# biiiipy/JaxMARL-HFT

Hardware: AMD Instinct MI355X
Metric: env steps/sec (whole node), 2-agent MARL, 10-level LOB, NUM_ENVS=4096 (higher is better)
Workload: dtype int32

## Files before the change

### jaxmarl-hft_amd/csrc/hftlob.hip

```cpp
#include <hip/hip_runtime.h>
#include <stdint.h>
#include <string.h>
#include <stdio.h>
#include <mutex>
#include <type_traits>
#include <limits.h>

#include "../../include/hftlob.h"

typedef int32_t i32;
typedef uint32_t u32;
typedef uint8_t u8;
#define DEV __device__ __forceinline__

DEV int lane_id() { return __lane_id(); }
DEV i32 rdl(i32 v, int l) { return __builtin_amdgcn_readlane(v, l); }
DEV i32 wrl(i32 old, i32 val, int l) { return __lane_id() == l ? val : old; }
DEV i32 uni(i32 v) { return __builtin_amdgcn_readfirstlane(v); }
DEV float unif(float v) { return __int_as_float(__builtin_amdgcn_readfirstlane(__float_as_int(v))); }
DEV i32 wadd(i32 a, i32 b) { return (i32)((u32)a + (u32)b); }
DEV i32 wsub(i32 a, i32 b) { return (i32)((u32)a - (u32)b); }
DEV i32 wmul(i32 a, i32 b) { return (i32)((u32)a * (u32)b); }
DEV i32 iabs_(i32 a) { return a < 0 ? wsub(0, a) : a; }
DEV i32 isign(i32 a) { return (a > 0) - (a < 0); }
// ... 2370 lines not shown
}
DEV Key lane_key(Key v) { return Key{(u32)rdl((i32)v.a, 0), (u32)rdl((i32)v.b, 0)}; }
DEV Key from_lane(Key v, int src) {
    return Key{(u32)__builtin_amdgcn_ds_bpermute(src << 2, (i32)v.a), (u32)__builtin_amdgcn_ds_bpermute(src << 2, (i32)v.b)};
}
template <bool MD>
DEV StepKeys step_keys(const hftlob_env_cfg& c, int n_env, int e, const u32* keys, bool sampled, const Key& master) {
    const bool part = c.prng_partitionable;
    const int l = lane_id(), nTy = c.n_types, A = c.n_action_msgs;
    Key key;
    Key nm{0u, 0u};
    if (sampled) {
        const Key v = split_key(master, n_env + 1, l == 0 ? e + 1 : 0, part);
        key = lane_key(v);
        nm = Key{(u32)rdl((i32)v.a, 1), (u32)rdl((i32)v.b, 1)};
    } else {
        key = Key{keys[2 * e], keys[2 * e + 1]};
    }
    const bool two = part && c.n_agents <= 16 && A <= 32;
    const bool hi_lane = two && l >= 48;
    const int ag = l - (hi_lane ? 48 : 32);
    int t = 0, i = 0;
    agent_of_lane(c, ag < 0 ? 0 : ag, t, i);
    const bool agent_lane = (ag >= 0) & (ag < c.n_agents);
    const Key L1 = split_key(key, l < 2 ? 2 : nTy, l < 2 ? l : l - 2, part);
    StepKeys o;
    o.key = key;
    o.next_master = nm;
    o.k1 = Key{(u32)rdl((i32)L1.a, 0), (u32)rdl((i32)L1.b, 0)};
    o.key_reset = Key{(u32)rdl((i32)L1.a, 1), (u32)rdl((i32)L1.b, 1)};
    if (two) {
        const Key P2 = from_lane(L1, agent_lane ? 2 + t : 0);
        const Key L2 = split_key(P2, agent_lane ? type_n_agents(c, t) : 2, agent_lane ? i : 1, part);
        const Key L3 = split_key(L2, 2, ((l == 0) | hi_lane) ? 1 : 0, part);
        const Key sub = from_lane(L3, 0);
        const u32 bits = random_bits(l < A ? sub : L3, 1, l < A ? l : 0, part);
        o.shuffle_bits = bits;
        const u32 hb = bits, lb = (u32)__builtin_amdgcn_ds_bpermute(((l + 16) & 63) << 2, (i32)bits);
        const i32 na = agent_lane ? type_action_hi(c, t, MD) : 1;
        const u32 span = na <= 0 ? 1u : (u32)na;
        u32 mult = 65536u % span;
        mult = (mult * mult) % span;
        o.acts = (i32)(((hb % span) * mult + (lb % span)) % span);
        return o;
    }
    const Key P2 = from_lane(L1, agent_lane ? 2 + t : 0);
    const Key L2 = split_key(P2, agent_lane ? type_n_agents(c, t) : 2, agent_lane ? i : 1, part);
    const Key L3a = split_key(L2, 2, l == 0 ? 1 : 0, part);
    const Key L3b = split_key(L2, 2, 1, part);
    const Key sub = from_lane(L3a, 0);
    o.shuffle_bits = random_bits(sub, A > 0 ? A : 1, l < A ? l : 0, part);
    const u32 hb = random_bits(L3a, 1, 0, part), lb = random_bits(L3b, 1, 0, part);
    const i32 na = agent_lane ? type_action_hi(c, t, MD) : 1;
    const u32 span = na <= 0 ? 1u : (u32)na;
    u32 mult = 65536u % span;
    mult = (mult * mult) % span;
    o.acts = (i32)(((hb % span) * mult + (lb % span)) % span);
    return o;
}

#define KB_STEPS 4
__host__ __device__ inline bool kb_ok(const hftlob_env_cfg& c) {
    return c.prng_partitionable && c.n_agents <= 3 && c.n_action_msgs <= 8 && c.n_types <= 6 &&
           6 + c.n_agents + c.n_action_msgs <= 16;
}
__host__ __device__ inline int kb_words(const hftlob_env_cfg& c) { return 6 + c.n_agents + c.n_action_msgs; }
__host__ __device__ inline bool rows_in_trades(const hftlob_env_cfg& c, int nT) {
    const int ar = c.n_cancel_msgs + c.n_action_msgs;
    return ar <= 128 && 8 * ar <= 8 * nT + PAD_SCR;
}
struct LdsMap {
    int rows, axs, book, kb, words;
};
__host__ __device__ inline LdsMap lds_map(const hftlob_env_cfg& c, int nO, int nT, bool alias) {
    LdsMap m;
    const int rw = alias ? 0 : (c.n_cancel_msgs + c.n_action_msgs) * 8;
    m.axs = rw;
    m.book = rw + ((c.n_agents * 6 + 3) & ~3);
    m.rows = alias ? m.book + 12 * nO : 0;
    m.kb = m.book + book_words(nO, nT);
    m.words = m.kb + (kb_ok(c) ? KB_STEPS * kb_words(c) : 0);
    return m;
}
template <bool MD>
DEV void step_keys_batch(const hftlob_env_cfg& c, int n_env, int e, Key& mk, int nb, i32* kb) {
    const bool part = true;
    const int l = lane_id(), ll = l & 15, j = l >> 4, nTy = c.n_types, A = c.n_action_msgs, KW = kb_words(c);
    i32 ka = 0, kb2 = 0;
#pragma unroll 1
    for (int q = 0; q < nb; ++q) {
        const Key v = split_key(mk, n_env + 1, l == 1 ? e + 1 : 0, part);
        ka = wlane(ka, rdl((i32)v.a, 1), 16 * q);
        kb2 = wlane(kb2, rdl((i32)v.b, 1), 16 * q);
        mk = Key{(u32)rdl((i32)v.a, 0), (u32)rdl((i32)v.b, 0)};
    }
    const int b0 = l & ~15;
    const Key key{(u32)__builtin_amdgcn_ds_bpermute(b0 << 2, ka), (u32)__builtin_amdgcn_ds_bpermute(b0 << 2, kb2)};
    const bool hi_lane = ll >= 12;
    const int ag = ll - (hi_lane ? 12 : 8);
    int t = 0, i = 0;
    agent_of_lane(c, ag < 0 ? 0 : ag, t, i);
    const bool agent_lane = (ll >= 8) & (ag >= 0) & (ag < c.n_agents);
    const Key L1 = split_key(key, ll < 2 ? 2 : nTy, ll < 2 ? ll : ll - 2, part);
    const Key P2 = from_lane(L1, b0 + (agent_lane ? 2 + t : 0));
    const Key L2 = split_key(P2, agent_lane ? type_n_agents(c, t) : 2, agent_lane ? i : 1, part);
    const Key L3 = split_key(L2, 2, ((ll == 0) | hi_lane) ? 1 : 0, part);
    const Key sub = from_lane(L3, b0);
    const u32 bits = random_bits(ll < A ? sub : L3, 1, ll < A ? ll : 0, part);
    const u32 hb = bits, lb = (u32)__builtin_amdgcn_ds_bpermute(((l + 4) & 63) << 2, (i32)bits);
    const i32 na = agent_lane ? type_action_hi(c, t, MD) : 1;
    const u32 span = na <= 0 ? 1u : (u32)na;
    u32 mult = 65536u % span;
    mult = (mult * mult) % span;
    const i32 act = (i32)(((hb % span) * mult + (lb % span)) % span);
    const i32 l1a = __builtin_amdgcn_ds_bpermute((b0 + ((ll >> 2) & 1)) << 2, (i32)L1.a);
    const i32 l1b = __builtin_amdgcn_ds_bpermute((b0 + ((ll >> 2) & 1)) << 2, (i32)L1.b);
    const i32 ac = __builtin_amdgcn_ds_bpermute((b0 + 8 + (ll >= 6 ? ll - 6 : 0)) << 2, act);
    const i32 sh = __builtin_amdgcn_ds_bpermute((b0 + (ll >= 6 + c.n_agents ? ll - 6 - c.n_agents : 0)) << 2, (i32)bits);
    i32 w = ll == 0 ? (i32)key.a : (ll == 1 ? (i32)key.b : ((ll & 1) ? l1b : l1a));
    w = ll >= 6 + c.n_agents ? sh : (ll >= 6 ? ac : w);
    if ((j < nb) & (ll < KW)) kb[j * KW + ll] = w;
    wave_sync();
}
DEV StepKeys load_keys(const hftlob_env_cfg& c, const i32* row) {
    const int l = lane_id(), na = c.n_agents, A = c.n_action_msgs;
    StepKeys o;
    o.key = Key{(u32)uni(row[0]), (u32)uni(row[1])};
    o.k1 = Key{(u32)uni(row[2]), (u32)uni(row[3])};
    o.key_reset = Key{(u32)uni(row[4]), (u32)uni(row[5])};
    o.next_master = Key{0u, 0u};
    const int ag = l - 32;
    o.acts = ((ag >= 0) & (ag < na)) ? row[6 + (ag < 0 ? 0 : ag)] : 0;
    o.shuffle_bits = l < A ? (u32)row[6 + na + (l < A ? l : 0)] : 0u;
    return o;
}

DEV void fixed_time_mask(int4& x, int4& y, i32 t_end) {
    if (y.z >= t_end) {
        x = make_int4(0, 0, 0, 0);
        y.x = 0;
        y.y = 0;
    }
}

template <bool BID, int S>
DEV i32 l2_side(const Side<S>& s, int R, const Valid<S>& V, i32 maxint, i32 outv) {
    const int l = lane_id();
    i32 x[S], q[S];
    ldcol(s.t, R, FQ, q);
#pragma unroll
    for (int r = 0; r < S; ++r) x[r] = BID ? wmul(-1, s.pc[r]) : (s.pc[r] == -1 ? maxint : s.pc[r]);
    i32 prev = 0;
    for (int k = 0; k < HFTLOB_L2_LEVELS; ++k) {
        i32 m = INT_MAX;
        lmask any = 0;
#pragma unroll
        for (int r = 0; r < S; ++r) {
            const bool ok = V.v[r] && (k == 0 || x[r] > prev);
            m = imin_(m, ok ? x[r] : INT_MAX);
            any |= bal(ok);
        }
        i32 lv = wave_min(m);
        if (any == 0ull) lv = BID ? 1 : -1;
        else prev = lv;
        i32 p = BID ? wmul(-1, lv) : lv;
        p = p == -1 ? (BID ? wsub(0, maxint) : maxint) : p;
// ... 135 lines not shown
        B.a.rp = B.a.rq = B.b.rp = B.b.rq = 0;
        for (int k = 0; k < cnt; ++k) {
            if (!((skip >> k) & 1ull)) {
                const i32 h = rdl(hx, k), d2 = rdl(x.z, k), d3 = rdl(x.w, k), d4 = rdl(y.x, k), d5 = rdl(y.y, k),
                          d6 = rdl(y.z, k), d7 = rdl(y.w, k);
                const i32 ntr0 = B.ntr;
                if (RC) B.mi = base + k;
                if ((i32)B.fl >= 0) process_msg_<false, RC>(B, (u32)k, h, x.y, d2, d3, d4, d5, d6, d7);
                else process_msg_<true, RC>(B, (u32)k, h, x.y, d2, d3, d4, d5, d6, d7);
                refresh_best(B, (u32)k);
#ifdef HFTLOB_DEPTH_BOTH
                (void)ntr0;
                dirty = 3u;
#else
                const i32 kind = h & H_KIND;
                const bool add = kind <= H_BID;
                const bool no_trade = (ntr0 >= 0) & (ntr0 < B.c.nT) & (B.ntr == ntr0) & (d6 != -1);
                dirty |= ((kind == H_ASK) | (kind == H_CNL_ASK)) ? 1u : 2u;
                if (add & !no_trade) dirty = 3u;
#endif
            }
            const int j = base + k - first_kept;
            if (j >= 0) {
                if (gd) {
                    if (dirty & 1u) dv = depth_side<false>(B.a, R, B.vs, B.c.maxint, n_levels, dv);
                    if (dirty & 2u) dv = depth_side<true>(B.b, R, B.vs, B.c.maxint, n_levels, dv);
                    dirty = 0u;
                    if (l < dw) gd[(size_t)j * dw + l] = dv;
                }
                if (gsa) {
                    store_side(B.a, gsa + (size_t)j * R * 6, R, B.vs);
                    store_side(B.b, gsb + (size_t)j * R * 6, R, B.vs);
                }
            }
        }
    }
    store_side(B.a, ga, R, B.vs);
    store_side(B.b, gb, R, B.vs);
    store_trades(B.tr, gt, B.vt);
}

#define MAX_AGENT_ROWS 128

constexpr u32 INFO_F32_MM = 0xC0B9FFu, INFO_F32_EXE = 0x13Cu;
constexpr u32 TALLY_SUM_LANES = 0x34u;
struct TallyLane { double a, b; };
DEV int tally_word(int l) { return l < 25 ? 8 + 2 * l : (l < 40 ? l - 32 : 58 + 2 * (l - 40)); }
DEV TallyLane tally_load(const double* row, bool all) {
    const int l = lane_id();
    const bool hdr = (l >= 32) & (l < 40);
    TallyLane t{0.0, 0.0};
    if ((l < 25) | hdr | ((l >= 40) & all)) {
        const int w = tally_word(l);
        t.a = row[w];
        t.b = row[hdr ? (((TALLY_SUM_LANES >> (l - 32)) & 1u) ? 2 : 3) : w + 1];
    }
    return t;
}
DEV void tally_store(double* row, const TallyLane& t, float rew, const i32 (&iw)[HFTLOB_INFO_AGENT_WORDS], u32 f32,
                     bool all) {
    const int l = lane_id();
    const int k = l < 25 ? l - 1 : l - 40;
    i32 v = 0;
#pragma unroll
    for (int j = 0; j < HFTLOB_INFO_AGENT_WORDS; ++j) v = k == j ? iw[j] : v;
    double x = ((f32 >> (k & 31)) & 1u) ? (double)bitf(v) : (double)v;
    if (l == 0) x = (double)rew;
    if ((l >= 32) & (l < 40)) {
        const int h = l - 32;
        const double run = t.b + (((TALLY_SUM_LANES >> h) & 1u) ? (double)rew : 1.0);
        double a;
        if (h == 0) a = t.a + 1.0;
        else if (h == 1) a = t.a + (all ? 1.0 : 0.0);
        else if (h < 4) a = all ? 0.0 : run;
        else if ((h & 1) == 0) a = all ? t.a + run : t.a;
        else a = all ? t.a + run * run : t.a;
        row[h] = a;
    } else if ((l < 25) | ((l >= 40) & all)) {
        const int w = tally_word(l);
        row[w] = t.a + x;
        row[w + 1] = t.b + x * x;
    }
}
template <int S, int NFIX, bool RC, bool RA = false, bool QUIET = false, int PK = -1, bool TALLY = false>
DEV bool env_step_dev(const hftlob_env_cfg& c, int key_n, int ek, int e, const u32* __restrict__ keys, bool master,
                      Key& mk,
                      i32* __restrict__ actions_io, const i32* __restrict__ msg_data,
                      const i32* __restrict__ init_states, i32* __restrict__ state, float* __restrict__ obs_out,
                      float* __restrict__ rew_out, u8* __restrict__ done_all_out, u8* __restrict__ dones_out,
                      i32* __restrict__ info_out, i32* __restrict__ obs_raw_out, i32* __restrict__ msgs_out,
                      i32* __restrict__ debug_out, i32* lds, bool resident, bool keep, u32& fl_carry,
                      const i32* pre_keys = nullptr, bool emit_rt = true, double* __restrict__ stats = nullptr,
                      int act_e = -1) {
    const bool emit = !QUIET && emit_rt;
    const bool vals = TALLY || emit;
    STAMP(t_start);
#ifdef HFTLOB_STAMPS
    const unsigned long long rt_start = __builtin_amdgcn_s_memrealtime();
#endif
    const int l = lane_id();
    const int M = c.n_msgs, D = c.n_data_msg, A = c.n_action_msgs, C = c.n_cancel_msgs;
    i32* rec = state + (size_t)e * c.rec_words;
    Book<S> B;
    B.c = lobcfg(c.lob);
    if (NFIX > 0) { B.c.nO = NFIX; B.c.nT = NFIX; }
    const int R = B.c.nO;
    const LdsMap LM = lds_map(c, B.c.nO, B.c.nT, RA);
    i32* rows = lds + LM.rows;
    i32* axs = lds + LM.axs;
    book_bind(B, lds + LM.book);
    SideRows<S> fa, fb;
    if (!resident) {
        fetch_side(fa, rec + c.off_asks, B.vs);
        fetch_side(fb, rec + c.off_bids, B.vs);
    }
    const int naw = c.rec_words - c.off_agents;
    const bool agw_pre = naw <= 64;
    const i32 agw = (agw_pre & (l < naw)) ? rec[c.off_agents + l] : 0;
    const bool batched = PK == 1 || (PK < 0 && pre_keys);
    const StepKeys SK = batched ? load_keys(c, pre_keys) : step_keys<NFIX == 0>(c, key_n, ek, keys, master, mk);
    if (master && !batched) mk = SK.next_master;
    const Key key_reset = SK.key_reset;
    if (RC) {
        B.ek = c.shuffle_action_messages ? split_key(SK.k1, 2, 0, c.prng_partitionable) : SK.k1;
        B.nmsg = M;
        B.part = c.prng_partitionable;
    }
    SUBSTAMP(t_keys);
    const i32* Lr = rec + c.off_loaded;
    const i32* Wr = rec + c.off_world;
    const i32 ld_t0 = Lr[LD_T0], win = Lr[LD_WIN], max_steps = Lr[LD_MAXS], start_index = Lr[LD_START],
              step = Lr[LD_STEP];
    const i32 wt0 = Wr[W_T0], wt1 = Wr[W_T1], oidc = Wr[W_OIDC];
    const float wmid = bitf(Wr[W_MID]);
    const i32 old_last_ba = rec[c.off_best_asks + (M - 1) * 2], old_last_bb = rec[c.off_best_bids + (M - 1) * 2];
    bool excl_any = false, excl_cfg = false;
    for (int t = 0; t < c.n_types; ++t) {
        const bool ex = c.types[t].kind == HFTLOB_AGENT_MM && c.types[t].exclude_extreme_spreads;
        excl_cfg |= ex;
        if (vals && ex) {
            bool any = false;
            for (int m = l; m < M; m += 64) {
                const i32 pa = rec[c.off_best_asks + m * 2], pb = rec[c.off_best_bids + m * 2];
                any |= (i2f(wsub(pa, pb)) / (i2f(wadd(pa, pb)) / 2.0f)) > 0.1f;
            }
            excl_any = ballot(any) != 0ull;
        }
    }
    const bool store_best = NFIX == 0 || (!keep | excl_cfg);
    i32 dstart = wadd(start_index, wmul(D, step));
    dstart = imax_(0, imin_(dstart, c.n_data_rows - D));
    const bool ftime = NFIX == 0 && c.ep_type == 1;
    const i32 t_end = wadd(ld_t0, c.episode_time);
    int4 px = make_int4(0, 0, 0, 0), py = px;
    if ((l >= C + A) & (l < M)) {
        const i32* g = msg_data + (size_t)(dstart + l - (C + A)) * 8;
        ld_msg(g, px, py);
        if (ftime) fixed_time_mask(px, py, t_end);
    }
    if (resident) {
        relink_side(B.a, R, B.vs);
        relink_side(B.b, R, B.vs);
        B.fl = fl_carry | F_STALE_A | F_STALE_B | STALE_ANY;
    } else {
        B.fl = commit_side<true>(B.a, fa, R, B.vs) | commit_side<false>(B.b, fb, R, B.vs) | F_STALE_A | F_STALE_B | STALE_ANY;
        B.fl |= slow_bit(B.fl);
    }
    SUBSTAMP(t_load);

#ifdef HFTLOB_STAMPS
    unsigned long long acc_act = 0, acc_cnl = 0, acc_flt = 0, acc_mmr = 0, acc_exr = 0, acc_obs = 0;
#endif
    constexpr bool REG = NFIX > 0 && !RA;
    RegRows<S> sink;
    if constexpr (REG) {
        SUBSTAMP(tc0);
        sink.init(B.a.t, B.b.t, R, C, wt0, wt1);
        STAMP_ACC(acc_cnl, tc0);
    }
    const auto srows = row_sink<REG>(sink, rows);
    {
        int ag = 0, arow = C, crow = 0, aw = 0;
        const i32* st = rec + c.off_agents;
        for (int t = 0; t < c.n_types; ++t) {
            const hftlob_agent_type_cfg& tc = c.types[t];
            for (int i = 0; i < tc.n_agents; ++i, ++ag) {
                const i32 tid = wsub(tc.trader_id0, i);
                const int w = tc.action_width;
                i32* aio = actions_io ? actions_io + (size_t)(act_e < 0 ? e : act_e) * c.action_words + aw : nullptr;
                aw += w;
                i32 act, av[4] = {0, 0, 0, 0};
                if (NFIX > 0 || w == 1) {
                    if (master) {
                        act = rdl(SK.acts, 32 + ag);
                        if (aio && l == 0) aio[0] = act;
                    } else {
                        act = aio[0];
                    }
                    av[0] = act;
                } else {
                    i32 v = 0;
                    if (master) {
                        const bool part = c.prng_partitionable;
                        const Key ka = split_key(split_key(SK.key, c.n_types, t, part), tc.n_agents, i, part);
                        v = randint_vec(ka, w, l < w ? l : 0, 0, action_hi(tc), part);
                        if (aio && l < w) aio[l] = v;
                    } else if (l < w) {
                        v = aio[l];
                    }
#pragma unroll
                    for (int j = 0; j < 4; ++j) av[j] = rdl(v, j);
                    act = av[0];
                }
                i32 s4[4];
                {
                    const int b = (int)(st - (rec + c.off_agents));
#pragma unroll
                    for (int k = 0; k < 4; ++k) s4[k] = agw_pre ? rdl(agw, b + k) : st[k];
// ... 147 lines not shown
        if (act_lane) {
#pragma unroll
            for (int k = 0; k < 8; ++k) rows[(C + dest) * 8 + k] = f[k];
        }
        wave_sync();
    }

    STAMP(t_agents);
    if (!RA) trades_fill(B.tr, B.vt, -1);
    B.ntr = 0;
    const int AR = C + A;
    bool abort_any = false;
    i32 prev_a = -1, prev_b = -1;
    float mid_acc = 0.0f, pa_acc = 0.0f, pb_acc = 0.0f;
    i32 last_p_a = 0, last_p_b = 0, last_t0 = 0, last_t1 = 0;
    int4 nx = px, ny = py;
    if constexpr (REG) {
        if (l < AR) { nx = sink.x; ny = sink.y; }
    }
#ifndef HFTLOB_NO_CARRY
    i32* carry = B.filt - PAD_FILT + PAD_CARRY;
    if (!RA && resident) {
        const i32 v = carry[l & 15];
        B.a.best_p = rdl(v, 0); B.a.best_q = rdl(v, 1); B.a.xp = rdl(v, 2); B.a.top = rdl(v, 3);
        B.a.top_p = rdl(v, 4); B.a.top_ts = rdl(v, 5); B.a.top_tns = rdl(v, 6);
        B.b.best_p = rdl(v, 7); B.b.best_q = rdl(v, 8); B.b.top = rdl(v, 9); B.b.top_p = rdl(v, 10);
        B.b.top_ts = rdl(v, 11); B.b.top_tns = rdl(v, 12);
        B.fl &= ~(F_STALE_A | F_STALE_B | STALE_ANY);
    }
#endif
#ifdef HFTLOB_STAMPS_CHUNK
    unsigned long long acc_dec = 0, acc_pre = 0, acc_loop = 0, acc_post = 0;
#endif
    for (int base = 0; base < M; base += 64) {
#ifdef HFTLOB_STAMPS_CHUNK
        const unsigned long long tc0 = __builtin_amdgcn_s_memtime();
#endif
        const int row = base + l;
        int4 x = nx, y = ny;
        if (REG) {
        } else if (RA ? (base == 0) & (row < AR) : row < AR) {
            x = reinterpret_cast<const int4*>(rows + row * 8)[0];
            y = reinterpret_cast<const int4*>(rows + row * 8)[1];
        } else if (ftime && base > 0 && row >= AR) {
            fixed_time_mask(x, y, t_end);
        }
        if (msgs_out && row < M) {
            int4* mo = reinterpret_cast<int4*>(msgs_out + ((size_t)e * M + row) * 8);
            mo[0] = x;
            mo[1] = y;
        }
        {
            const bool nv = (row + 64 >= AR) & (row + 64 < M);
            ld_msg(msg_data + (size_t)(dstart + (nv ? row + 64 - AR : 0)) * 8, nx, ny);
        }
        if (RA && (base == 0)) {
            if (row + 64 < AR) {
                nx = reinterpret_cast<const int4*>(rows + (row + 64) * 8)[0];
                ny = reinterpret_cast<const int4*>(rows + (row + 64) * 8)[1];
            }
            wave_sync();
            trades_fill(B.tr, B.vt, -1);
        }
        decode_msgs(B.c, x, y);
        i32 rpa = 0, rqa = 0, rpb = 0, rqb = 0;
        const int cnt = uni(imin_(64, M - base));
#ifdef HFTLOB_STAMPS_CHUNK
        acc_dec += __builtin_amdgcn_s_memtime() - tc0;
#endif
        run_chunk<RC>(B, x, y, cnt, base, rpa, rqa, rpb, rqb CHUNK_ARGS);
#ifdef HFTLOB_STAMPS_CHUNK
        const unsigned long long tc1 = __builtin_amdgcn_s_memtime();
#endif
        abort_any |= bal((l < cnt) & ((rpa == -1) | (rpb == -1))) != 0ull;
        i32 pa = rpa, pb = rpb;
        if ((base == 0) & (l == 0)) {
            pa = pa == -1 ? old_last_ba : pa;
            pb = pb == -1 ? old_last_bb : pb;
        }
        const i32 caq = rpa == -1 ? 0 : rqa, cbq = rpb == -1 ? 0 : rqb;
        const i32 cap = ffill(pa, prev_a), cbp = ffill(pb, prev_b);
        prev_a = rdl(cap, cnt - 1);
        prev_b = rdl(cbp, cnt - 1);
        if ((row < M) & (store_best | (row == M - 1))) {
            reinterpret_cast<int2*>(rec + c.off_best_asks)[row] = make_int2(cap, caq);
            reinterpret_cast<int2*>(rec + c.off_best_bids)[row] = make_int2(cbp, cbq);
        }
        if (row < M) {
            const float mf = i2f(wadd(cbp, cap)) / 2.0f;
            mid_acc = base == 0 ? mf : mid_acc + mf;
            if (info_out) {
                pa_acc = base == 0 ? i2f(cap) : pa_acc + i2f(cap);
                pb_acc = base == 0 ? i2f(cbp) : pb_acc + i2f(cbp);
            }
        }
        if (base + 64 >= M) {
            last_t0 = rdl(y.z, cnt - 1);
            last_t1 = rdl(y.w, cnt - 1);
        }
#ifdef HFTLOB_STAMPS_CHUNK
        acc_post += __builtin_amdgcn_s_memtime() - tc1;
#endif
    }
    last_p_a = prev_a;
    last_p_b = prev_b;
#ifndef HFTLOB_NO_CARRY
    if (!RA && keep) {
        i32 v = B.a.best_p;
        v = wlane(v, B.a.best_q, 1); v = wlane(v, B.a.xp, 2); v = wlane(v, B.a.top, 3); v = wlane(v, B.a.top_p, 4);
        v = wlane(v, B.a.top_ts, 5); v = wlane(v, B.a.top_tns, 6); v = wlane(v, B.b.best_p, 7);
        v = wlane(v, B.b.best_q, 8); v = wlane(v, B.b.top, 9); v = wlane(v, B.b.top_p, 10);
        v = wlane(v, B.b.top_ts, 11); v = wlane(v, B.b.top_tns, 12);
        if (l < 13) carry[l] = v;
    }
#endif
    StepCtx X;
    X.avg_mid = wave_fsum(mid_acc) / (float)M;
    X.last_ba = last_p_a; X.last_bb = last_p_b;
    X.last_mid = i2f(wadd(last_p_b, last_p_a)) / 2.0f;
    X.wmid = wmid;
    X.old_last_ba = old_last_ba; X.old_last_bb = old_last_bb;
    X.init0 = ld_t0; X.step = step;
    X.ep_done = wsub(wsub(max_steps, step), 1) <= 1;
    const bool all = X.ep_done;

    STAMP(t_book);
    WorldView wv;
    wv.best_ask_p = last_p_a; wv.best_bid_p = last_p_b;
    wv.vol_a = wv.vol_b = 0;
    if (emit) { wv.vol_a = side_volume(B.a, R, B.vs); wv.vol_b = side_volume(B.b, R, B.vs); }
    if (debug_out) write_debug(B, debug_out + (size_t)e * HFTLOB_DEBUG_WORDS(B.c.nT));
    if (keep) fl_carry = B.fl;
    if (!all & !keep) {
        store_side(B.a, rec + c.off_asks, R, B.vs);
        store_side(B.b, rec + c.off_bids, R, B.vs);
        store_trades(B.tr, rec + c.off_trades, B.vt);
    }
    wv.step = wadd(step, 1); wv.max_steps = max_steps; wv.mid = X.last_mid;
    wv.t0 = last_t0; wv.t1 = last_t1; wv.it0 = ld_t0; wv.it1 = Lr[LD_T1];
    const float dt = i2f(last_t0) + i2f(last_t1) / 1e9f - i2f(wt0) - i2f(wt1) / 1e9f;
    wv.dt = dt;
    i32* info = info_out ? info_out + (size_t)e * c.info_words : nullptr;
    if (vals | !all) {
        TradeView<S> TV;
        {
            const i32 ovr0[8] = {0, 0, 0, 0, 0, 0, 0, 0};
            trade_view(B, TV, false, -1, ovr0);
        }
        int ag = 0;
        i32* st = rec + c.off_agents;
        for (int t = 0; t < c.n_types; ++t) {
            const hftlob_agent_type_cfg& tc = c.types[t];
            for (int i = 0; i < tc.n_agents; ++i, ++ag) {
                const i32 tid = wsub(tc.trader_id0, i);
                const int nw = agent_words(tc);
                i32 s[13];
                {
                    const int b = (int)(st - (rec + c.off_agents));
                    for (int k = 0; k < 13; ++k) s[k] = k < nw ? (agw_pre ? rdl(agw, b + k) : st[k]) : 0;
                }
                i32 d = 0;
                float rew;
                TallyLane tl{0.0, 0.0};
#ifndef HFTLOB_KO_TALLY
                if constexpr (TALLY) tl = tally_load(stats + ((size_t)e * c.n_agents + ag) * HFTLOB_EVAL_WORDS, all);
#endif
                i32 iw[HFTLOB_INFO_AGENT_WORDS];
                for (int k = 0; k < HFTLOB_INFO_AGENT_WORDS; ++k) iw[k] = 0;
                ActX ax1;
                ax1.bid_price = uni(axs[ag * 6 + 0]); ax1.ask_price = uni(axs[ag * 6 + 1]);
                ax1.bid_dist = uni(axs[ag * 6 + 2]); ax1.ask_dist = uni(axs[ag * 6 + 3]);
                ax1.bid_quant = uni(axs[ag * 6 + 4]); ax1.ask_quant = uni(axs[ag * 6 + 5]);
                SUBSTAMP(tr0);
                if (tc.kind == HFTLOB_AGENT_MM) {
                    MMRew R;
#if defined(HFTLOB_KO_REWARD) || defined(HFTLOB_KO_MM_REWARD)
                    memset(&R, 0, sizeof R);
#else
                    mm_reward(c, tc, B, X, s, tid, excl_any, TV, R, vals);
#endif
                    STAMP_ACC(acc_mmr, tr0);
                    const float tot = bitf(s[3]) + R.PnL;
                    s[0] = ax1.bid_dist; s[1] = ax1.ask_dist; s[2] = R.end_inventory; s[3] = fbit(tot);
                    s[4] = fbit(R.cash);
                    rew = R.reward / tc.reward_scaling_quo;
                    iw[0] = fbit(R.reward); iw[1] = fbit(R.reward_pv); iw[2] = fbit(R.reward_spooner);
                    iw[3] = fbit(R.end_of_ep_pv); iw[4] = fbit(R.reward_spooner_damped);
                    iw[5] = fbit(R.reward_spooner_asym_damped); iw[6] = fbit(R.reward_spooner_asym_damped2);
                    iw[7] = fbit(R.reward_delta_pv); iw[8] = fbit(tot); iw[9] = 0; iw[10] = s[2];
                    iw[11] = fbit(R.delta_mid); iw[12] = fbit(R.market_share); iw[13] = fbit(R.buyPnL);
                    iw[14] = R.forced_unwind; iw[15] = fbit(R.invPnL); iw[16] = ax1.bid_price;
                    iw[17] = ax1.ask_price; iw[18] = ax1.bid_dist; iw[19] = ax1.ask_dist;
                    iw[20] = ax1.ask_quant; iw[21] = ax1.bid_quant; iw[22] = fbit(R.sellPnL);
                    iw[23] = fbit(R.inventoryValue);
                } else {
                    EXRew R;
#if defined(HFTLOB_KO_REWARD) || defined(HFTLOB_KO_EXE_REWARD)
                    memset(&R, 0, sizeof R);
#else
                    exe_reward(c, tc, B, X, s, tid, TV, R, vals);
#endif
                    STAMP_ACC(acc_exr, tr0);
                    s[2] = wadd(s[2], R.agentQuant);
                    s[4] = fbit(R.p_vwap);
                    s[5] = fbit(bitf(s[5]) + i2f(R.qp_agent));
                    s[6] = fbit(bitf(s[6]) + R.drift);
                    s[7] = fbit(bitf(s[7]) + R.advantage);
                    s[8] = fbit(R.slippage_rm); s[9] = fbit(R.price_adv_rm); s[10] = fbit(R.price_drift_rm);
                    s[11] = fbit(R.vwap_rm); s[12] = fbit(R.trade_duration);
                    d = wsub(s[1], s[2]) <= 0;
                    rew = R.reward / tc.reward_scaling_quo;
                    iw[0] = R.quant_left; iw[1] = d; iw[2] = fbit(R.slippage); iw[3] = fbit(R.vwap_rm);
                    iw[4] = fbit(R.drift); iw[5] = fbit(R.advantage); iw[6] = R.doom_quant; iw[7] = s[3];
                    iw[8] = fbit(R.reward_info);
                }
#ifndef HFTLOB_KO_TALLY
                if constexpr (TALLY)
                    tally_store(stats + ((size_t)e * c.n_agents + ag) * HFTLOB_EVAL_WORDS, tl, rew, iw,
                                tc.kind == HFTLOB_AGENT_MM ? INFO_F32_MM : INFO_F32_EXE, all);
#endif
                if (emit & (l == 0)) {
                    rew_out[(size_t)e * c.n_agents + ag] = rew;
                    dones_out[(size_t)e * c.n_agents + ag] = (u8)(d != 0);
                }
                if (info) {
                    i32 v = 0;
                    for (int k = 0; k < HFTLOB_INFO_AGENT_WORDS; ++k) if (l == k) v = iw[k];
                    if (l < HFTLOB_INFO_AGENT_WORDS) info[HFTLOB_INFO_WORLD_WORDS + ag * HFTLOB_INFO_AGENT_WORDS + l] = v;
                }
                SUBSTAMP(to0);
                if (!all) {
                    i32 v = 0;
                    for (int k = 0; k < 13; ++k) if (l == k) v = s[k];
                    if (l < nw) st[l] = v;
#ifndef HFTLOB_KO_OBS
                    if (emit)
                        write_obs<false>(c, tc, wv, s, obs_out + ((size_t)e * c.n_agents + ag) * c.obs_stride, d != 0,
                                         ftime);
#endif
                }
                if (obs_raw_out)
                    write_obs<true>(c, tc, wv, s, obs_raw_out + ((size_t)e * c.n_agents + ag) * c.obs_stride, false,
                                    ftime);
                STAMP_ACC(acc_obs, to0);
                st += nw;
            }
        }
    }
    STAMP(t_rewards);
    const float new_mid = X.last_mid;
    if (info) {
        const float ava = wave_fsum(pa_acc) / (float)M, avb = wave_fsum(pb_acc) / (float)M;
        i32 wv_[HFTLOB_INFO_WORLD_WORDS] = {win, fbit(new_mid), wadd(step, 1), last_t0, last_t1, wsub(oidc, A),
                                            last_p_a, last_p_b, fbit(ava), fbit(avb), fbit(dt), (i32)X.ep_done,
                                            (i32)abort_any, wsub(last_p_a, last_p_b)};
        i32 v = 0;
        for (int k = 0; k < HFTLOB_INFO_WORLD_WORDS; ++k) if (l == k) v = wv_[k];
        if (l < HFTLOB_INFO_WORLD_WORDS) info[l] = v;
    }
    if (emit & (l == 0)) done_all_out[e] = (u8)all;
#ifdef HFTLOB_STAMPS
    if (info && l == 0) {
        const unsigned long long t_end = __builtin_amdgcn_s_memtime();
        info[0] = (i32)(t_agents - t_start); info[1] = (i32)(t_book - t_agents);
        info[2] = (i32)(t_rewards - t_book); info[3] = (i32)(t_end - t_rewards); info[4] = (i32)all;
#ifndef HFTLOB_STAMPS_COARSE
        info[5] = (i32)(t_keys - t_start); info[6] = (i32)(t_load - t_keys); info[7] = (i32)(t_rows - t_load);
        info[8] = (i32)(t_agents - t_rows);
#else
        info[5] = info[6] = info[7] = info[8] = 0;
        (void)t_keys; (void)t_load; (void)t_rows;
#endif
#ifdef HFTLOB_STAMPS_CHUNK
        info[9] = (i32)acc_dec; info[10] = (i32)acc_pre; info[11] = (i32)acc_loop; info[12] = (i32)acc_post;
        info[13] = 0; info[14] = 0;
        (void)acc_act; (void)acc_cnl; (void)acc_flt; (void)acc_mmr; (void)acc_exr; (void)acc_obs;
#else
        info[9] = (i32)acc_act; info[10] = (i32)acc_cnl; info[11] = (i32)acc_flt;
        info[12] = (i32)acc_mmr; info[13] = (i32)acc_exr; info[14] = (i32)acc_obs;
#endif
        info[15] = (i32)(__builtin_amdgcn_s_memrealtime() - rt_start);
    }
#endif
    if (all) {
        env_reset_dev<S>(c, key_reset, init_states, rec, emit ? obs_out + (size_t)e * c.n_agents * c.obs_stride : nullptr,
                         B.vs, B.vt, ftime);
        return true;
    }
    if (l == 0) {
        rec[c.off_loaded + LD_STEP] = wadd(step, 1);
        i32* W = rec + c.off_world;
        W[W_T0] = last_t0; W[W_T1] = last_t1; W[W_OIDC] = wsub(oidc, A); W[W_MID] = fbit(new_mid); W[W_DT] = fbit(dt);
    }
    return false;
}

template <int S, int NFIX, bool RC, bool RA = false>
__global__ __launch_bounds__(64) void k_env_step(hftlob_env_cfg c, int n_env, int key_e0, int key_n,
                                                 const u32* __restrict__ keys, const u32* __restrict__ master,
                                                 u32* __restrict__ master_out, i32* __restrict__ actions_io,
                                                 const i32* __restrict__ msg_data, const i32* __restrict__ init_states,
                                                 i32* __restrict__ state, hftlob_step_out out) {
    one_wave();
    extern __shared__ __attribute__((aligned(16))) i32 lds[];
    const int e = blockIdx.x;
    if (e >= n_env) return;
    Key mk{0u, 0u};
    if (master) mk = Key{master[0], master[1]};
    u32 fl = 0;
    env_step_dev<S, NFIX, RC, RA>(c, key_n, key_e0 + e, e, keys, master != nullptr, mk, actions_io, msg_data, init_states,
                              state, out.obs, out.rewards, out.done_all, out.dones, out.info, out.obs_raw, out.msgs,
                              out.debug, lds, false, false, fl);
    if (master && (e == 0) && (lane_id() == 0)) { master_out[0] = mk.a; master_out[1] = mk.b; }
}

typedef const __attribute__((address_space(4))) hftlob_env_cfg kcfg_t;

#define WAVE_SLOTS (8 * 16 * 16 * 64)
static __device__ unsigned long long g_wave_eta[WAVE_SLOTS];
DEV unsigned long long* wave_row(u32 hwid, u32 xcc, u32& slot) {
    const u32 cu = ((xcc & 7u) * 16u + ((hwid >> 13) & 7u) * 2u + ((hwid >> 12) & 1u)) * 16u + ((hwid >> 8) & 15u);
    slot = ((hwid >> 4) & 3u) * 16u + (hwid & 15u);
    return g_wave_eta + (size_t)cu * 64u;
}
#ifndef HFTLOB_PRIO_SCOPE
#define HFTLOB_PRIO_SCOPE __HIP_MEMORY_SCOPE_WORKGROUP
#endif
DEV void balance_prio(unsigned long long* row, u32 slot, unsigned long long r0, int done, int left) {
    const int l = lane_id();
    const unsigned long long now = __builtin_amdgcn_s_memrealtime();
    const float el = (float)(now - r0);
    const unsigned long long eta = now + (unsigned long long)(el * ((float)left / (float)done));
    if (l == 0) __hip_atomic_store(row + slot, eta, __ATOMIC_RELAXED, HFTLOB_PRIO_SCOPE);
    unsigned long long v = __hip_atomic_load(row + l, __ATOMIC_RELAXED, HFTLOB_PRIO_SCOPE);
    v = (u32)l == slot ? eta : v;
    v = ((u32)l >> 4) == (slot >> 4) ? v : 0ull;
    const lmask live = bal(v > now);
    const lmask later = live & bal((v > eta) | ((v == eta) & ((u32)l < slot)));
    const int n = __builtin_popcountll(live), rank = __builtin_popcountll(later);
    const int q = n > 0 ? (4 * rank) / n : 0;
    if (q == 0) __builtin_amdgcn_s_setprio(3);
    else if (q == 1) __builtin_amdgcn_s_setprio(2);
    else if (q == 2) __builtin_amdgcn_s_setprio(1);
    else __builtin_amdgcn_s_setprio(0);
}
template <int S, int NFIX, bool RC, bool RA = false, int KB = -1>
__global__ __launch_bounds__(64, 4) void k_env_rollout(hftlob_env_cfg c, int n_env, int key_e0, int key_n, int n_steps,
                                                    int per_step, const u32* __restrict__ master,
                                                    u32* __restrict__ master_out, i32* __restrict__ actions_io,
                                                    const i32* __restrict__ msg_data,
                                                    const i32* __restrict__ init_states, i32* __restrict__ state,
                                                    hftlob_step_out out) {
    one_wave();
    extern __shared__ __attribute__((aligned(16))) i32 lds[];
    const int e = blockIdx.x;
    if (e >= n_env) return;
    Key mk{master[0], master[1]};
    kcfg_t* kp = (kcfg_t*)__builtin_amdgcn_kernarg_segment_ptr();
    bool resident = false;
    u32 fl = 0;
#ifndef HFTLOB_NO_BALANCE
    const unsigned long long bal_r0 = __builtin_amdgcn_s_memrealtime();
    const u32 bal_hwid = __builtin_amdgcn_s_getreg(0xF804), bal_xcc = __builtin_amdgcn_s_getreg(0x7814);
    u32 bal_slot;
    unsigned long long* bal_row = wave_row(bal_hwid, bal_xcc, bal_slot);
#endif
#ifdef HFTLOB_WAVETIME
    const unsigned long long wt_start = __builtin_amdgcn_s_memtime(), wt_rstart = __builtin_amdgcn_s_memrealtime();
    const u32 wt_hwid = __builtin_amdgcn_s_getreg(0xF804), wt_xcc = __builtin_amdgcn_s_getreg(0x7814);
#endif
    const bool kbat = KB < 0 ? kb_ok(c) : KB == 1;
    const int kbw = kb_words(c);
    i32* kbuf = lds + lds_map(c, NFIX > 0 ? NFIX : c.lob.n_orders, NFIX > 0 ? NFIX : c.lob.n_trades, RA).kb;
    auto step = [&](auto Q, int t) {
        constexpr bool QT = decltype(Q)::value;
        const size_t o = per_step ? (size_t)t * n_env : 0;
        const int tb = t % KB_STEPS;
        kcfg_t* cp = kp;
        i32* st = state;
        const i32* md = msg_data;
        const i32* is = init_states;
        asm volatile("" : "+s"(cp), "+s"(st), "+s"(md), "+s"(is));
        const hftlob_env_cfg& cc = *(const hftlob_env_cfg*)cp;
        STAMP(kb0);
        if (kbat && tb == 0) step_keys_batch<NFIX == 0>(cc, key_n, key_e0 + e, mk, imin_(KB_STEPS, n_steps - t), kbuf);
        STAMP(kb1);
        const bool ox = !QT;
#ifdef HFTLOB_STAMPS_QUIET
        const bool ox_info = true;
#else
        const bool ox_info = ox;
#endif
        const bool reset = env_step_dev<S, NFIX, RC, RA, QT, KB>(
            cc, key_n, key_e0 + e, e, nullptr, true, mk, actions_io ? actions_io + o * cc.action_words : nullptr, md,
            is, st, out.obs + o * cc.n_agents * cc.obs_stride, out.rewards + o * cc.n_agents, out.done_all + o,
            out.dones + o * cc.n_agents, ox_info && out.info ? out.info + o * cc.info_words : nullptr,
            ox && out.obs_raw ? out.obs_raw + o * cc.n_agents * cc.obs_stride : nullptr,
            ox && out.msgs ? out.msgs + o * cc.n_msgs * 8 : nullptr,
            ox && out.debug ? out.debug + o * (size_t)HFTLOB_DEBUG_WORDS(cc.lob.n_trades) : nullptr, lds,
            NFIX > 0 && resident, NFIX > 0 && t + 1 < n_steps, fl, kbat ? kbuf + tb * kbw : nullptr, !QT);
        resident = uni(!reset) != 0;
        STAMP(bp0);
#ifndef HFTLOB_NO_BALANCE
#ifndef HFTLOB_BALANCE_EVERY
#define HFTLOB_BALANCE_EVERY 1
#endif
#ifndef HFTLOB_BALANCE_MIN_ENVS
#define HFTLOB_BALANCE_MIN_ENVS 1024
#endif
        if ((t + 1 < n_steps) && ((t % HFTLOB_BALANCE_EVERY) == 0) && (n_env > HFTLOB_BALANCE_MIN_ENVS))
            balance_prio(bal_row, bal_slot, bal_r0, t + 1, n_steps - t - 1);
#endif
#ifdef HFTLOB_STAMPS
        if (out.info && per_step && lane_id() == 0) {
            i32* irow = out.info + ((size_t)t * n_env + e) * cc.info_words;
            irow[16] = (i32)(kb1 - kb0);
            irow[17] = (i32)(__builtin_amdgcn_s_memtime() - bp0);
        }
#endif
#ifdef HFTLOB_WAVETIME
        if (out.info && per_step) {
            const unsigned long long now = __builtin_amdgcn_s_memtime(), rnow = __builtin_amdgcn_s_memrealtime();
            const i32 w10[10] = {(i32)(u32)now, (i32)(u32)(now >> 32), (i32)wt_hwid, (i32)wt_xcc, (i32)(u32)wt_start,
                                 (i32)(u32)(wt_start >> 32), (i32)(u32)rnow, (i32)(u32)(rnow >> 32),
                                 (i32)(u32)wt_rstart, (i32)(u32)(wt_rstart >> 32)};
            i32 v = 0;
#pragma unroll
            for (int k = 0; k < 10; ++k) v = lane_id() == k ? w10[k] : v;
            if (lane_id() < 10) out.info[((size_t)t * n_env + e) * cc.info_words + lane_id()] = v;
        }
#endif
    };
    int t = 0;
#ifdef HFTLOB_STAMPS_QUIET
    if (true) {
#else
    if (!per_step) {
#endif
#pragma unroll 1
        for (; t + 1 < n_steps; ++t) step(std::integral_constant<bool, true>{}, t);
    }
#pragma unroll 1
    for (; t < n_steps; ++t) step(std::integral_constant<bool, false>{}, t);
#ifndef HFTLOB_NO_BALANCE
    if (lane_id() == 0) __hip_atomic_store(bal_row + bal_slot, __builtin_amdgcn_s_memrealtime(), __ATOMIC_RELAXED,
                                           HFTLOB_PRIO_SCOPE);
#endif
    if ((e == 0) && (lane_id() == 0)) { master_out[0] = mk.a; master_out[1] = mk.b; }
}

template <int S, int NFIX, bool RC, bool RA = false>
__global__ __launch_bounds__(64, 4) void k_env_rollout_actions(hftlob_env_cfg c, int n_env, int n_steps, int per_step,
                                                            const u32* __restrict__ keys,
                                                            const i32* __restrict__ actions,
                                                            const i32* __restrict__ msg_data,
                                                            const i32* __restrict__ init_states,
                                                            i32* __restrict__ state, hftlob_step_out out) {
    one_wave();
    extern __shared__ __attribute__((aligned(16))) i32 lds[];
    const int e = blockIdx.x;
    if (e >= n_env) return;
    Key mk{0u, 0u};
    kcfg_t* kp = (kcfg_t*)__builtin_amdgcn_kernarg_segment_ptr();
    bool resident = false;
    u32 fl = 0;
#ifndef HFTLOB_NO_BALANCE
    const unsigned long long bal_r0 = __builtin_amdgcn_s_memrealtime();
    const u32 bal_hwid = __builtin_amdgcn_s_getreg(0xF804), bal_xcc = __builtin_amdgcn_s_getreg(0x7814);
    u32 bal_slot;
    unsigned long long* bal_row = wave_row(bal_hwid, bal_xcc, bal_slot);
#endif
    auto step = [&](auto Q, int t) {
        constexpr bool QT = decltype(Q)::value;
        const size_t o = per_step ? (size_t)t * n_env : 0;
        kcfg_t* cp = kp;
        i32* st = state;
        const i32* md = msg_data;
        const i32* is = init_states;
        asm volatile("" : "+s"(cp), "+s"(st), "+s"(md), "+s"(is));
        const hftlob_env_cfg& cc = *(const hftlob_env_cfg*)cp;
        const bool ox = !QT;
        const bool reset = env_step_dev<S, NFIX, RC, RA, QT, 0>(
            cc, n_env, e, e, keys + (size_t)t * n_env * 2, false, mk,
// ... 666 lines not shown
```

Measured before the change: 92.53 million.

## Carry per-env scalar and agent state in LDS across quiet resident steps

In the fused multi-step kernel's quiet path, the per-env loaded/world scalars, the last best ask/bid, and the agent state words are now kept in an LDS scratch row between consecutive steps. Each step then reads them from LDS and lane reads instead of global memory, and skips writing them back to global when another carried step follows. This removes small dependent global loads and stores on every step's critical path. The cost is extra template complexity and a correctness dependence on the final step and resets writing state back to global correctly.

```diff
diff --git a/jaxmarl-hft_amd/csrc/hftlob.hip b/jaxmarl-hft_amd/csrc/hftlob.hip
--- a/jaxmarl-hft_amd/csrc/hftlob.hip
+++ b/jaxmarl-hft_amd/csrc/hftlob.hip
@@ -2476,6 +2476,12 @@
     m.words = m.kb + (kb_ok(c) ? KB_STEPS * kb_words(c) : 0);
     return m;
 }
+constexpr int SC_AGW = 64, SC_WORDS = SC_AGW + 16;
+enum { SC_LD_T0 = 0, SC_WIN, SC_MAXS, SC_START, SC_STEP, SC_W_T0, SC_W_T1, SC_OIDC, SC_MID, SC_OLD_BA, SC_OLD_BB, SC_N };
+static_assert(SC_N <= SC_WORDS - SC_AGW, "the carried scalars fit their 16-word row");
+__host__ __device__ inline bool state_carry_ok(const hftlob_env_cfg& c, int nO, int nT) {
+    return c.rec_words - c.off_agents <= SC_AGW && SC_WORDS <= lds_map(c, nO, nT, false).axs;
+}
 template <bool MD>
 DEV void step_keys_batch(const hftlob_env_cfg& c, int n_env, int e, Key& mk, int nb, i32* kb) {
     const bool part = true;
@@ -2777,7 +2783,7 @@
         row[w + 1] = t.b + x * x;
     }
 }
-template <int S, int NFIX, bool RC, bool RA = false, bool QUIET = false, int PK = -1, bool TALLY = false>
+template <int S, int NFIX, bool RC, bool RA = false, bool QUIET = false, int PK = -1, bool TALLY = false, bool SC = false>
 DEV bool env_step_dev(const hftlob_env_cfg& c, int key_n, int ek, int e, const u32* __restrict__ keys, bool master,
                       Key& mk,
                       i32* __restrict__ actions_io, const i32* __restrict__ msg_data,
@@ -2786,7 +2792,7 @@
                       i32* __restrict__ info_out, i32* __restrict__ obs_raw_out, i32* __restrict__ msgs_out,
                       i32* __restrict__ debug_out, i32* lds, bool resident, bool keep, u32& fl_carry,
                       const i32* pre_keys = nullptr, bool emit_rt = true, double* __restrict__ stats = nullptr,
-                      int act_e = -1) {
+                      int act_e = -1, bool sc_keep = false) {
     const bool emit = !QUIET && emit_rt;
     const bool vals = TALLY || emit;
     STAMP(t_start);
@@ -2811,7 +2817,20 @@
     }
     const int naw = c.rec_words - c.off_agents;
     const bool agw_pre = naw <= 64;
-    const i32 agw = (agw_pre & (l < naw)) ? rec[c.off_agents + l] : 0;
+    bool sc_in = false, sc_out = false;
+    i32* scw = rows;
+    i32 sc_agw = 0, scv = 0;
+    if constexpr (SC) {
+        static_assert(NFIX > 0 && !RA, "the state carry lives in the rows region of the register-rows kernel");
+        const bool sc_ok = state_carry_ok(c, B.c.nO, B.c.nT);
+        sc_in = sc_ok & resident;
+        sc_out = sc_ok & keep & sc_keep;
+        if (sc_in) {
+            sc_agw = scw[l];
+            scv = scw[SC_AGW + (l & 15)];
+        }
+    }
+    const i32 agw = SC && sc_in ? sc_agw : (agw_pre & (l < naw)) ? rec[c.off_agents + l] : 0;
     const bool batched = PK == 1 || (PK < 0 && pre_keys);
     const StepKeys SK = batched ? load_keys(c, pre_keys) : step_keys<NFIX == 0>(c, key_n, ek, keys, master, mk);
     if (master && !batched) mk = SK.next_master;
@@ -2824,11 +2843,21 @@
     SUBSTAMP(t_keys);
     const i32* Lr = rec + c.off_loaded;
     const i32* Wr = rec + c.off_world;
-    const i32 ld_t0 = Lr[LD_T0], win = Lr[LD_WIN], max_steps = Lr[LD_MAXS], start_index = Lr[LD_START],
-              step = Lr[LD_STEP];
-    const i32 wt0 = Wr[W_T0], wt1 = Wr[W_T1], oidc = Wr[W_OIDC];
-    const float wmid = bitf(Wr[W_MID]);
-    const i32 old_last_ba = rec[c.off_best_asks + (M - 1) * 2], old_last_bb = rec[c.off_best_bids + (M - 1) * 2];
+    i32 ld_t0, win, max_steps, start_index, step, wt0, wt1, oidc, old_last_ba, old_last_bb;
+    float wmid;
+    if (SC && sc_in) {
+        ld_t0 = rdl(scv, SC_LD_T0); win = rdl(scv, SC_WIN); max_steps = rdl(scv, SC_MAXS);
+        start_index = rdl(scv, SC_START); step = rdl(scv, SC_STEP);
+        wt0 = rdl(scv, SC_W_T0); wt1 = rdl(scv, SC_W_T1); oidc = rdl(scv, SC_OIDC);
+        wmid = bitf(rdl(scv, SC_MID));
+        old_last_ba = rdl(scv, SC_OLD_BA); old_last_bb = rdl(scv, SC_OLD_BB);
+    } else {
+        ld_t0 = Lr[LD_T0]; win = Lr[LD_WIN]; max_steps = Lr[LD_MAXS]; start_index = Lr[LD_START];
+        step = Lr[LD_STEP];
+        wt0 = Wr[W_T0]; wt1 = Wr[W_T1]; oidc = Wr[W_OIDC];
+        wmid = bitf(Wr[W_MID]);
+        old_last_ba = rec[c.off_best_asks + (M - 1) * 2]; old_last_bb = rec[c.off_best_bids + (M - 1) * 2];
+    }
     bool excl_any = false, excl_cfg = false;
     for (int t = 0; t < c.n_types; ++t) {
         const bool ex = c.types[t].kind == HFTLOB_AGENT_MM && c.types[t].exclude_extreme_spreads;
@@ -3142,7 +3171,12 @@
         const i32 cap = ffill(pa, prev_a), cbp = ffill(pb, prev_b);
         prev_a = rdl(cap, cnt - 1);
         prev_b = rdl(cbp, cnt - 1);
-        if ((row < M) & (store_best | (row == M - 1))) {
+        if constexpr (SC) {
+            if ((row < M) & (store_best | ((row == M - 1) & !sc_out))) {
+                reinterpret_cast<int2*>(rec + c.off_best_asks)[row] = make_int2(cap, caq);
+                reinterpret_cast<int2*>(rec + c.off_best_bids)[row] = make_int2(cbp, cbq);
+            }
+        } else if ((row < M) & (store_best | (row == M - 1))) {
             reinterpret_cast<int2*>(rec + c.off_best_asks)[row] = make_int2(cap, caq);
             reinterpret_cast<int2*>(rec + c.off_best_bids)[row] = make_int2(cbp, cbq);
         }
@@ -3292,7 +3326,13 @@
                 if (!all) {
                     i32 v = 0;
                     for (int k = 0; k < 13; ++k) if (l == k) v = s[k];
-                    if (l < nw) st[l] = v;
+                    if constexpr (SC) {
+                        if (sc_out) {
+                            if (l < nw) scw[(int)(st - (rec + c.off_agents)) + l] = v;
+                        } else if (l < nw) {
+                            st[l] = v;
+                        }
+                    } else if (l < nw) st[l] = v;
 #ifndef HFTLOB_KO_OBS
                     if (emit)
                         write_obs<false>(c, tc, wv, s, obs_out + ((size_t)e * c.n_agents + ag) * c.obs_stride, d != 0,
@@ -3346,6 +3386,17 @@
         env_reset_dev<S>(c, key_reset, init_states, rec, emit ? obs_out + (size_t)e * c.n_agents * c.obs_stride : nullptr,
                          B.vs, B.vt, ftime);
         return true;
+    }
+    if constexpr (SC) {
+        if (sc_out) {
+            i32 v = ld_t0;
+            v = wlane(v, win, SC_WIN); v = wlane(v, max_steps, SC_MAXS); v = wlane(v, start_index, SC_START);
+            v = wlane(v, wadd(step, 1), SC_STEP); v = wlane(v, last_t0, SC_W_T0); v = wlane(v, last_t1, SC_W_T1);
+            v = wlane(v, wsub(oidc, A), SC_OIDC); v = wlane(v, fbit(new_mid), SC_MID);
+            v = wlane(v, last_p_a, SC_OLD_BA); v = wlane(v, last_p_b, SC_OLD_BB);
+            if (l < SC_N) scw[SC_AGW + l] = v;
+            return false;
+        }
     }
     if (l == 0) {
         rec[c.off_loaded + LD_STEP] = wadd(step, 1);
@@ -3451,14 +3502,20 @@
 #else
         const bool ox_info = ox;
 #endif
-        const bool reset = env_step_dev<S, NFIX, RC, RA, QT, KB>(
+#ifdef HFTLOB_NO_STATE_CARRY
+        constexpr bool SCQ = false;
+#else
+        constexpr bool SCQ = QT && NFIX > 0 && !RA;
+#endif
+        const bool reset = env_step_dev<S, NFIX, RC, RA, QT, KB, false, SCQ>(
             cc, key_n, key_e0 + e, e, nullptr, true, mk, actions_io ? actions_io + o * cc.action_words : nullptr, md,
             is, st, out.obs + o * cc.n_agents * cc.obs_stride, out.rewards + o * cc.n_agents, out.done_all + o,
             out.dones + o * cc.n_agents, ox_info && out.info ? out.info + o * cc.info_words : nullptr,
             ox && out.obs_raw ? out.obs_raw + o * cc.n_agents * cc.obs_stride : nullptr,
             ox && out.msgs ? out.msgs + o * cc.n_msgs * 8 : nullptr,
             ox && out.debug ? out.debug + o * (size_t)HFTLOB_DEBUG_WORDS(cc.lob.n_trades) : nullptr, lds,
-            NFIX > 0 && resident, NFIX > 0 && t + 1 < n_steps, fl, kbat ? kbuf + tb * kbw : nullptr, !QT);
+            NFIX > 0 && resident, NFIX > 0 && t + 1 < n_steps, fl, kbat ? kbuf + tb * kbw : nullptr, !QT, nullptr, -1,
+            QT && t + 2 < n_steps);
         resident = uni(!reset) != 0;
         STAMP(bp0);
 #ifndef HFTLOB_NO_BALANCE
```

Result: no change. 92.80 million (median of 2 runs) (+0.3%).
